# taconite/arah-release

Measured on AMD Instinct MI355X. Metric: rendered rays/sec, higher is better.
Workload: dtype f32 (operands as hi+lo f16 pairs on the f16 MFMA pipe, fp32 accumulate)

## Files before the change

arah_release_amd/csrc/arah_hip.hip:

```cpp
#include <hip/hip_runtime.h>
#include <stdint.h>
#include <stdlib.h>
#include <string.h>

#include <atomic>
#include <mutex>

#include "../../include/arah_hip.h"
#include "pointwise.hpp"
#include "mlp.hpp"

using namespace arah;

namespace {

constexpr float kRootThresh = 1e-5f;
constexpr int kSphereIters = 50;
constexpr float kSurfaceRange = 0.05f;
constexpr float kClampDist = 0.1f;
constexpr int kBroydenSteps = 50;
constexpr float kDvg = 1.0f;
constexpr int kMaxVerts = 6912;
constexpr int kKnnThreads = 1024;
constexpr int kMaxGrid = 512;
// ... 1863 lines not shown
    }
    append_ids(keep, i, list, count);
}

__global__ void k_joint_seam_out(int n, const float* xbest, const float* zbest, const float* err_best, const uint8_t* valid,
                                 float* x, float* z, uint8_t* conv) {
    const int i = blockIdx.x * blockDim.x + threadIdx.x;
    if (i >= n) return;
    x[(size_t)i * 3] = xbest[(size_t)i * 3];
    x[(size_t)i * 3 + 1] = xbest[(size_t)i * 3 + 1];
    x[(size_t)i * 3 + 2] = xbest[(size_t)i * 3 + 2];
    z[i] = zbest[i];
    conv[i] = (valid[i] != 0 && err_best[i] < kRootThresh) ? 1 : 0;
}

__global__ void k_trace_finalize(FrameDev fr, int n, const float* near_far, const float* xbest, const float* zbest,
                                 const float* err_best, float* points_hat_norm, uint8_t* conv, float* start,
                                 float* end) {
    const BodyConst bc = load_bc(fr);
    const int i = blockIdx.x * blockDim.x + threadIdx.x;
    if (i >= n) return;
    const float nr = near_far[i * 2], fa = near_far[i * 2 + 1];
    const float z = zbest[i];
    const bool c = (err_best[i] < kRootThresh) && (z >= nr) && (z <= fa);
    const V3 xn = normalize_pt(bc, V3{xbest[(size_t)i * 3], xbest[(size_t)i * 3 + 1], xbest[(size_t)i * 3 + 2]});
    points_hat_norm[(size_t)i * 3] = xn.x;
    points_hat_norm[(size_t)i * 3 + 1] = xn.y;
    points_hat_norm[(size_t)i * 3 + 2] = xn.z;
    conv[i] = c ? 1 : 0;
    start[i] = c ? z : nr;
    end[i] = fa;
}

#include "finish.hpp"

template <typename F>
__device__ __forceinline__ float jittered(F val, int i, int m, float t) {
    const float v = val(i);
    const float lower = i == 0 ? v : 0.5f * (v + val(i - 1));
    const float upper = i == m - 1 ? v : 0.5f * (val(i + 1) + v);
    return lower + (upper - lower) * t;
}

__global__ void k_sample_depths(int n, int S, int n_near, int n_far, const float* near_far, const uint8_t* conv,
                                const float* start, const float* end, const float* lin_s, const float* lin_near,
                                const float* lin_far, const float* rand_s, const float* rand_near,
                                const float* rand_far, float* z, uint8_t* mask) {
    const int i = blockIdx.x * blockDim.x + threadIdx.x;
    if (i >= n) return;
    const float st = start[i], en = end[i];
    float* zr = z + (size_t)i * S;
    uint8_t* mr = mask + (size_t)i * S;
    auto uni = [&](int s) { return st + (en - st) * lin_s[s]; };
    auto uni_j = [&](int s) { return rand_s ? jittered(uni, s, S, rand_s[(size_t)i * S + s]) : uni(s); };
    if (!conv[i] || (n_near <= 0 && n_far <= 0)) {
        for (int s = 0; s < S; ++s) {
            zr[s] = uni_j(s);
            mr[s] = 1;
        }
        return;
    }
    const int nc = n_near + 1 + n_far;
    const float base = st - kSurfaceRange;
    const float nb = near_far[i * 2];
    const float span = fmaxf(st - kSurfaceRange - nb, 1e-5f);
    auto surf = [&](int a) { return base + (kSurfaceRange * 2.0f) * lin_near[a]; };
    auto farv = [&](int b) { return nb + span * lin_far[b]; };
// ... 594 lines not shown
    w.u_Jinv = c.take<float>(N * 16);
    w.err_best_ray = c.take<float>(N);
    w.xbest_ray = c.take<float>(N * 3);
    w.zbest_ray = c.take<float>(N);
    w.o_xnorm = c.take<float>(N * 3);
    w.o_Tray = c.take<float>(N * 16);
    w.o_start = c.take<float>(N);
    w.o_end = c.take<float>(N);
    w.o_acc = c.take<float>(N);
    w.o_conv = c.take<uint8_t>(N);
    w.listA = c.take<int>(Q);
    w.listB = c.take<int>(Q);
    w.q_err = c.take<float>(Q);
    w.o_z = c.take<float>(Q);
    w.o_pts = c.take<float>(Q * 3);
    w.o_T = c.take<float>(Q * 16);
    w.o_mask = c.take<uint8_t>(Q);
    w.q_smask = c.take<uint8_t>(Q);
    w.shaded = c.take<f32x4>(Q);
    w.listC = c.take<int>(Q);
    w.listD = c.take<int>(Q);
    w.tcounts = c.take<int>(TC_COUNT);
    w.ray_tier = c.take<uint8_t>(N);
    w.bytes = align_up(c.off, 256);
    return w;
}

struct Knobs {
    int max_grid;
    int knn_group;
    int knn_below[3];
    int joint_bulk;
    int trace_bulk;
    int trace_small;
    bool train_b3;
    int canon_tier_wgs;
    int posed_canon;
};
inline const Knobs& knobs() {
    static const Knobs k = [] {
        auto env_int = [](const char* name, int dflt) {
            const char* e = getenv(name);
            return e ? atoi(e) : dflt;
        };
        Knobs v;
        const int g = env_int("ARAH_MAX_GRID", kMaxGrid);
        v.max_grid = g >= 1 && g <= kMaxGrid ? g : kMaxGrid;
        v.knn_group = env_int("ARAH_KNN_GROUP", 1);
        v.knn_below[0] = env_int("ARAH_KNN_WAVE_POINTS", 4096);
        v.knn_below[1] = env_int("ARAH_KNN_WAVE_RAYS", v.knn_group ? (1 << 30) : 32768);
        v.knn_below[2] = env_int("ARAH_KNN_WAVE_SAMPLES", 32768);
        v.joint_bulk = max(1, min(kBroydenSteps + 1, env_int("ARAH_JOINT_BULK_ITERS", 3)));
        v.trace_bulk = max(0, min(kSphereIters, env_int("ARAH_TRACE_BULK_STEPS", 24)));
        v.trace_small = env_int("ARAH_TRACE_SMALL", 4096);
        v.canon_tier_wgs = max(0, env_int("ARAH_CANON_TIER_WGS", 0));
        const char* ck = getenv("ARAH_CANON_KERNEL");
        v.posed_canon = !ck ? ARAH_CANON_KERNEL_WAVE : strcmp(ck, "tile") == 0 ? ARAH_CANON_KERNEL_TILE
                        : strcmp(ck, "wave_l2") == 0 ? ARAH_CANON_KERNEL_WAVE_L2 : ARAH_CANON_KERNEL_WAVE;
        const char* e = getenv("ARAH_TRAIN_ENGINE");
        v.train_b3 = !(e && strcmp(e, "fp32") == 0);
        return v;
    }();
    return k;
}

inline int grid_for(long long n_items, int per_block) {
    long long g = (n_items + per_block - 1) / per_block;
    if (g < 1) g = 1;
    const int cap = knobs().max_grid;
    if (g > cap) g = cap;
    return (int)g;
}

inline int check_launch() { return hipGetLastError() == hipSuccess ? ARAH_OK : ARAH_E_LAUNCH; }

inline int num_cus() {
    constexpr int kMaxDevices = 64;
    static std::atomic<int> cus[kMaxDevices];
    int dev = 0;
    if (hipGetDevice(&dev) != hipSuccess || dev < 0 || dev >= kMaxDevices) return 256;
    int v = cus[dev].load(std::memory_order_relaxed);
    if (v == 0) {
        if (hipDeviceGetAttribute(&v, hipDeviceAttributeMultiprocessorCount, dev) != hipSuccess || v <= 0) v = 256;
        cus[dev].store(v, std::memory_order_relaxed);
    }
    return v;
}
// ... 42 lines not shown
    if (done[dev].load(std::memory_order_relaxed)) return ARAH_OK;
    const int rc = setup_attributes_once();
    if (rc == ARAH_OK) done[dev].store(true, std::memory_order_release);
    return rc;
}

int setup_attributes_once() {
    bool failed = false;
    allow_lds(k_nearest_invlbs<SRC_POINTS>, kLdsKnn, failed);
    allow_lds(k_nearest_invlbs<SRC_RAYS>, kLdsKnn, failed);
    allow_lds(k_nearest_invlbs<SRC_SAMPLES>, kLdsKnn, failed);
    allow_lds(k_sdf_eval<false, false>, kLdsSdfFwd, failed);
    allow_lds(k_sdf_eval<false, true>, kLdsSdfFwd, failed);
    allow_lds(k_sdf_eval<true, false>, kLdsSdfGrad, failed);
    allow_lds(k_sdf_eval<true, true>, kLdsSdfGrad, failed);
    allow_lds(k_sdf_march<false>, kLdsSdfFwd, failed);
    allow_lds(k_sdf_march<true>, kLdsSdfFwd, failed);
    allow_lds(k_density<false>, kLdsSdfFwd, failed);
    allow_lds(k_density<true>, kLdsSdfFwd, failed);
    allow_lds(k_density<true, 8>, kLdsDensityWide, failed);
    allow_lds(k_sdf_lattice, kLdsDensityWide, failed);
    allow_lds(k_skin_eval, kLdsSkin, failed);
    allow_lds(k_skin_jac, kLdsSkin, failed);
    allow_lds(k_canon_solve<false>, kLdsCanonSolve, failed);
    allow_lds(k_canon_solve<true>, kLdsCanonSolve, failed);
    allow_lds((k_canon_wave<true, false>), kLdsCanonWave, failed);
    allow_lds((k_canon_wave<true, true>), kLdsCanonWave, failed);
    allow_lds((k_canon_wave<false, false>), kLdsCanonWave, failed);
    allow_lds((k_canon_wave<false, true>), kLdsCanonWave, failed);
    allow_lds(k_joint_iter<true, false>, kLdsJoint, failed);
    allow_lds(k_joint_iter<true, true>, kLdsJoint, failed);
    allow_lds(k_joint_iter<false, false>, kLdsJoint, failed);
    allow_lds(k_joint_iter<false, true>, kLdsJoint, failed);
    allow_lds(k_trace_finish<true>, kLdsTraceFinish, failed);
    allow_lds(k_trace_finish<false>, kLdsTraceFinish, failed);
    allow_lds(k_joint_finish<true>, kLdsJointFinish, failed);
    allow_lds(k_joint_finish<false>, kLdsJointFinish, failed);
    allow_lds(k_shade<false, false>, lds_shade<false>(), failed);
    allow_lds(k_shade<false, true>, lds_shade<false>(), failed);
    allow_lds(k_shade<true, false>, lds_shade<true>(), failed);
    allow_lds(k_shade<true, true>, lds_shade<true>(), failed);
    allow_lds((k_shade<false, true, true>), lds_shade_b3<false>(), failed);
    allow_lds((k_shade<true, true, true>), lds_shade_b3<true>(), failed);
    allow_lds((k_shade<false, false, false, true>), lds_shade<false>(), failed);
    allow_lds((k_shade<false, true, false, true>), lds_shade<false>(), failed);
    allow_lds((k_shade<true, false, false, true>), lds_shade<true>(), failed);
    allow_lds((k_shade<true, true, false, true>), lds_shade<true>(), failed);
    allow_lds((k_shade<false, true, true, true>), lds_shade_b3<false>(), failed);
    allow_lds((k_shade<true, true, true, true>), lds_shade_b3<true>(), failed);
    allow_lds(k_color_eval<false>, lds_color<false>(), failed);
    allow_lds(k_color_eval<true>, lds_color<true>(), failed);
    allow_lds(k_shade_train<false, false, false>, lds_shade_train<false>(), failed);
    allow_lds(k_shade_train<false, true, false>, lds_shade_train<false>(), failed);
    allow_lds(k_shade_train<true, false, false>, lds_shade_train<true>(), failed);
    allow_lds(k_shade_train<true, true, false>, lds_shade_train<true>(), failed);
    allow_lds(k_shade_train<false, false, true>, lds_shade_train<false>(), failed);
    allow_lds(k_shade_train<false, true, true>, lds_shade_train<false>(), failed);
    allow_lds(k_shade_train<true, false, true>, lds_shade_train<true>(), failed);
    allow_lds(k_shade_train<true, true, true>, lds_shade_train<true>(), failed);
    return failed ? ARAH_E_LAUNCH : ARAH_OK;
}


KnnData knn_of(const FrameDev& fd) {
    return KnnData{fd.knn.sorted4, fd.knn.spheres, reinterpret_cast<const GridInfo*>(fd.knn.grid), fd.knn.cells};
}

template <int SRC>
void launch_nearest(hipStream_t s, const FrameDev& fd, long long n_max, const float* pts, const RaySet& rs,
                    const float* depth, int n_steps, const int* list, const int* count, int n_direct, int* idx_out,
// ... 883 lines not shown
    int rc = run_broyden3(fd, w, tgt, CanonOut{x, T, w.q_err}, n, s, canon_kernel);
    if (rc) return rc;
    hipLaunchKernelGGL(k_broyden3_finalize, dim3((n + 255) / 256), dim3(256), 0, s, n, (const float*)w.q_err, err, conv);
    return check_launch();
}

static void joint_impl(const FrameDev& fd, Workspace& w, const RaySet& rs, int n, float* T, hipStream_t s) {
    int* cntB = w.counts + kNumCounts;
    const int gm = grid_for(n, kTile);
    hipLaunchKernelGGL(k_skin_jac, dim3(grid_for(n, 16)), dim3(kThreads), kLdsSkin, s, fd, (const float*)w.x0raw,
                       (const int*)w.listA, (const int*)&cntB[0], 0, w.jac_lbs, &w.ctr->n_skin_jac);
    LAUNCH_ENGINE(fd.split, (k_sdf_eval<true, true>), (k_sdf_eval<true, false>), dim3(gm), dim3(kThreads), kLdsSdfGrad, s,
                  fd, (const float*)w.xcur, (const int*)w.listA, (const int*)&cntB[0], 0, w.u_gx ,
                  (float*)nullptr, w.grad_sdf, w.spill, &w.ctr->n_sdf_fwd, &w.ctr->n_sdf_grad, 0);
    Broyden4State st{w.u_eval, w.u_step, w.u_gx, w.u_Jinv, w.err_best_ray, w.xbest_ray, w.zbest_ray, T};
    hipLaunchKernelGGL(k_joint_init, dim3(grid_for(n, 256)), dim3(256), 0, s, fd, st, rs, (const int*)w.listA,
                       (const int*)&cntB[0], (const float*)w.grad_sdf, (const float*)w.jac_lbs, (const float*)w.xcur,
                       (const float*)w.t, w.x0raw);
    const int bulk = knobs().joint_bulk;
    for (int it = 0; it < bulk; ++it) {
        int* lin = (it & 1) ? w.listB : w.listA;
        int* lout = (it & 1) ? w.listA : w.listB;
        if (it == 0)
            LAUNCH_ENGINE(fd.split, (k_joint_iter<true, true>), (k_joint_iter<true, false>), dim3(gm), dim3(kThreads),
                          kLdsJoint, s, fd, st, rs, (const int*)lin, (const int*)&cntB[it], lout, &cntB[it + 1],
                          &w.ctr->n_skin_fwd, &w.ctr->n_sdf_fwd);
        else
            LAUNCH_ENGINE(fd.split, (k_joint_iter<false, true>), (k_joint_iter<false, false>), dim3(gm), dim3(kThreads),
                          kLdsJoint, s, fd, st, rs, (const int*)lin, (const int*)&cntB[it], lout, &cntB[it + 1],
                          &w.ctr->n_skin_fwd, &w.ctr->n_sdf_fwd);
    }
    if (bulk <= kBroydenSteps) {
        const int* lin = (bulk & 1) ? w.listB : w.listA;
        const int gf = min(4 * num_cus(), max(1, (n + kFinTile - 1) / kFinTile));
        LAUNCH_ENGINE(fd.split, k_joint_finish<true>, k_joint_finish<false>, dim3(gf), dim3(kThreads), kLdsJointFinish, s, fd,
                      st, rs, lin, (const int*)&cntB[bulk], kBroydenSteps + 1 - bulk, &w.ctr->n_skin_fwd, &w.ctr->n_sdf_fwd);
    }
}

static int trace_impl(const ArahFrame* f, Workspace& w, const float* cam_loc, int32_t rays_per_cam,
                      const float* dirs, const float* near_far, int32_t n, int root_find_all, float* points_hat_norm,
                      float* T, uint8_t* conv, float* start, float* end, hipStream_t s, const uint8_t* skip = nullptr) {
    const FrameDev fd = to_dev(*f);
    const RaySet rs = make_rays(cam_loc, dirs, rays_per_cam);
    const int gb = (n + 255) / 256;
    int* cntA = w.counts;
    int* cntB = w.counts + kNumCounts;
    hipMemsetAsync(w.counts, 0, sizeof(int) * 3 * kNumCounts, s);
    hipMemsetAsync(w.nn_idx, 0xff, sizeof(int) * (size_t)n, s);
    hipLaunchKernelGGL(k_trace_begin, dim3(gb), dim3(256), 0, s, near_far, n, w.t, w.far, w.diverged, w.xcur, w.Tcur,
                       w.listA, &cntA[0], skip);
    TraceState ts{w.t, w.far, w.xcur, w.diverged};
    const int gm = grid_for(n, kTile);
    const int bulk = n <= knobs().trace_small ? 0 : knobs().trace_bulk;
    for (int it = 0; it < bulk; ++it) {
        int* lin = (it & 1) ? w.listB : w.listA;
        int* lout = (it & 1) ? w.listA : w.listB;
        launch_nearest<SRC_RAYS>(s, fd, n, (const float*)nullptr, rs, (const float*)w.t, 1, (const int*)lin,
                                 (const int*)&cntA[it], 0, w.nn_idx, w.xcur, w.Tcur, 0, &w.ctr->n_knn);
        LAUNCH_ENGINE(fd.split, k_sdf_march<true>, k_sdf_march<false>, dim3(gm), dim3(kThreads), kLdsSdfFwd, s, fd, ts,
                      (const int*)lin, (const int*)&cntA[it], lout, &cntA[it + 1], &w.ctr->n_sdf_fwd);
    }
    if (bulk < kSphereIters) {
        const int* lin = (bulk & 1) ? w.listB : w.listA;
        const int gf = min(4 * num_cus(), max(1, (n + kFinTile - 1) / kFinTile));
        LAUNCH_ENGINE(fd.split, k_trace_finish<true>, k_trace_finish<false>, dim3(gf), dim3(kThreads), kLdsTraceFinish, s, fd,
                      knn_of(fd), rs, ts, w.Tcur, w.nn_idx, lin, (const int*)&cntA[bulk], kSphereIters - bulk, &w.ctr->n_knn,
                      &w.ctr->n_sdf_fwd);
    }
    hipLaunchKernelGGL(k_joint_select, dim3(gb), dim3(256), 0, s, fd, n, (const float*)w.xcur, (const float*)w.Tcur,
                       (const float*)w.t, (const uint8_t*)w.diverged, root_find_all, w.x0raw, w.xbest_ray, w.zbest_ray, T,
                       w.err_best_ray, w.listA, &cntB[0]);
    joint_impl(fd, w, rs, n, T, s);
    hipLaunchKernelGGL(k_trace_finalize, dim3(gb), dim3(256), 0, s, fd, n, near_far, (const float*)w.xbest_ray,
                       (const float*)w.zbest_ray, (const float*)w.err_best_ray, points_hat_norm, conv, start, end);
    return check_launch();
}

int arah_trace(const ArahFrame* f, const float* cam_loc, int32_t rays_per_cam, const float* dirs,
               const float* near_far, int32_t n, int32_t root_find_all, float* points_hat_norm, float* T,
               uint8_t* conv, float* start, float* end, void* workspace, size_t wbytes, void* stream) {
    if (!f || n < 0 || !workspace) return ARAH_E_BADARG;
    if (n == 0) return ARAH_OK;
    if (!cam_loc || !dirs || !near_far || !points_hat_norm || !T || !conv || !start || !end) return ARAH_E_BADARG;
    Workspace w = carve(workspace, n, 1);
    if (wbytes < w.bytes) return ARAH_E_WORKSPACE;
    if (int arc = setup_attributes()) return arc;
    return trace_impl(f, w, cam_loc, rays_per_cam, dirs, near_far, n, root_find_all, points_hat_norm, T, conv, start,
                      end, reinterpret_cast<hipStream_t>(stream));
}

int arah_joint_root_find(const ArahFrame* f, const float* cam_loc, int32_t rays_per_cam, const float* dirs,
                         const uint8_t* valid, const float* x0, const float* z0, const float* T0, int32_t n, float* x,
                         float* z, float* T, uint8_t* conv, void* workspace, size_t wbytes, void* stream) {
    if (!f || n < 0 || !workspace) return ARAH_E_BADARG;
    if (n == 0) return ARAH_OK;
    if (!cam_loc || !dirs || !valid || !x0 || !z0 || !T0 || !x || !z || !T || !conv) return ARAH_E_BADARG;
    Workspace w = carve(workspace, n, 1);
    if (wbytes < w.bytes) return ARAH_E_WORKSPACE;
    if (int arc = setup_attributes()) return arc;
    hipStream_t s = reinterpret_cast<hipStream_t>(stream);
// ... 1334 lines not shown
```

arah_release_amd/csrc/finish.hpp:

```cpp
#pragma once

constexpr int kFinTile = 16;
constexpr size_t kLdsTraceFinish = (kFinTile * 4 * 2 + kFinTile * 16 + kFinTile * 8) * 4 + (size_t)kFinTile * kSdfLd * 4;
constexpr size_t kLdsJointFinish = (kFinTile * 4 * 3 + 24 * 16 + kFinTile * 2 + kFinTile * kLogitLd + 32) * 4 + (size_t)kFinTile * kSdfLd * 4;

template <bool SPLIT>
__global__ __launch_bounds__(kThreads, 4) void k_trace_finish(FrameDev fr, KnnData kd, RaySet rs, TraceState st, float* Tcur,
                                                            int* nn_idx, const int* list, const int* count, int steps_left,
                                                            unsigned long long* ctr_knn, unsigned long long* ctr_fwd) {
    const BodyConst bc = load_bc(fr);
    extern __shared__ __attribute__((aligned(16))) float smem[];
    float* xin = smem;
    float* outv = xin + kFinTile * 4;
    float* Tl = outv + kFinTile * 4;
    int* ids = reinterpret_cast<int*>(Tl + kFinTile * 16);
    float* tl = reinterpret_cast<float*>(ids + kFinTile);
    float* farl = tl + kFinTile;
    int* nnl = reinterpret_cast<int*>(farl + kFinTile);
    int* divl = nnl + kFinTile;
    int* s_live = divl + kFinTile;
    float* actA = reinterpret_cast<float*>(s_live + 3 * kFinTile);
    const int tid = threadIdx.x, wave = __builtin_amdgcn_readfirstlane(tid >> 6), lane = tid & 63;
    const int n = *count;
    const GridInfo g = *kd.grid;
    const float scale = sdf_scale(bc);
    int n_done = 0;
    for (int tile = blockIdx.x; tile * kFinTile < n; tile += gridDim.x) {
        __syncthreads();
        if (tid < kFinTile) {
            const int i = tile * kFinTile + tid;
            const int id = i < n ? list[i] : -1;
            ids[tid] = id;
            tl[tid] = id >= 0 ? st.t[id] : 0.f;
            farl[tid] = id >= 0 ? st.far[id] : 0.f;
            nnl[tid] = id >= 0 ? nn_idx[id] : -1;
            divl[tid] = 0;
        }
        for (int step = 0; step < steps_left; ++step) {
            __syncthreads();
            if (wave == 0) {
                const unsigned long long live = __ballot(lane < kFinTile && ids[lane] >= 0);
                n_done += __popcll(live);
                if (lane == 0) *s_live = live != 0ull;
            }
            __syncthreads();
            if (!*s_live) break;
            if (wave < 4) {
                const int s = wave * 4 + (lane >> 4);
                const int id = ids[s];
                if (id >= 0) {
                    const V3 p = ray_point(rs, id, tl[s]);
                    float best = 3.4e38f;
                    int bi = 0x7fffffff;
                    const int seed = nnl[s];
                    if (seed >= 0) {
                        const float dx = fr.verts_raw[seed * 3] - p.x, dy = fr.verts_raw[seed * 3 + 1] - p.y,
                                    dz = fr.verts_raw[seed * 3 + 2] - p.z;
                        best = dx * dx + dy * dy + dz * dz;
                        bi = seed;
                    }
                    bi = nearest_vertex_group16<kClusterSize>(kd, kd.sorted4, kd.spheres, g, p, best, bi, lane);
                    if ((lane & 15) == 0) {
                        float T[16];
                        vertex_transform(fr, bi, T);
                        const V3 y = V3{p.x - bc.trans[0], p.y - bc.trans[1], p.z - bc.trans[2]};
                        const V3 xh = normalize_pt(bc, inverse_affine_apply(T, y));
                        store_T(Tl + s * 16, T);
                        nnl[s] = bi;
                        reinterpret_cast<f32x4*>(xin)[s] = f32x4{xh.x, xh.y, xh.z, 0.f};
                    }
                } else if ((lane & 15) == 0) {
                    reinterpret_cast<f32x4*>(xin)[s] = f32x4{0.f, 0.f, 0.f, 0.f};
                }
            }
            __syncthreads();
            f32x4 dlast[kSdfMT][1];
            sdf_trunk<false, 1, SPLIT>(fr.sdf, xin, actA, kSdfLd, nullptr, dlast, wave, lane);
            sdf_head<SPLIT>(fr.sdf, actA, kSdfLd, outv, 4, tid, kFinTile);
            __syncthreads();
            if (tid < kFinTile) {
                const int id = ids[tid];
                if (id >= 0) {
                    const float sdf = outv[tid * 4] * scale;
                    const float march = fminf(fmaxf(sdf, -kClampDist), kClampDist);
                    bool div = false;
                    if (fabsf(march) > kRootThresh) {
                        const float t = tl[tid] + march;
                        tl[tid] = t;
                        div = t >= farl[tid];
                        divl[tid] = div ? 1 : 0;
                    }
                    const bool keep = !((fabsf(sdf) <= kRootThresh) || div);
                    if (!keep || step + 1 == steps_left) {
                        st.t[id] = tl[tid];
                        st.diverged[id] = divl[tid] ? 1 : 0;
                        const f32x4 xn = reinterpret_cast<const f32x4*>(xin)[tid];
                        st.xcur[(size_t)id * 3] = xn[0];
                        st.xcur[(size_t)id * 3 + 1] = xn[1];
                        st.xcur[(size_t)id * 3 + 2] = xn[2];
#pragma unroll
                        for (int c = 0; c < 4; ++c)
                            reinterpret_cast<f32x4*>(Tcur + (size_t)id * 16)[c] = reinterpret_cast<const f32x4*>(Tl + tid * 16)[c];
                        nn_idx[id] = nnl[tid];
                        ids[tid] = -1;
                    }
                }
            }
        }
    }
    if (tid == 0) {
        count_add(ctr_knn, n_done);
        count_add(ctr_fwd, n_done);
    }
}

template <bool SPLIT>
__global__ __launch_bounds__(kThreads, 4) void k_joint_finish(FrameDev fr, Broyden4State st, RaySet rs, const int* list,
                                                            const int* count, int iters_left, unsigned long long* ctr_skin,
                                                            unsigned long long* ctr_sdf) {
    const BodyConst bc = load_bc(fr);
    extern __shared__ __attribute__((aligned(16))) float smem[];
    constexpr int TW = kFinTile;
    float* xin = smem;
    float* xraw = xin + TW * 4;
    float* outv = xraw + TW * 4;
    float* sbones = outv + TW * 4;
    int* ids = reinterpret_cast<int*>(sbones + 24 * 16);
    int* s_live = ids + TW;
    float* logits = reinterpret_cast<float*>(s_live + TW);
    float* act = logits + TW * kLogitLd;
    const int tid = threadIdx.x, wave = __builtin_amdgcn_readfirstlane(tid >> 6), lane = tid & 63;
    const int n = *count;
    const float scale = sdf_scale(bc);
    int n_done = 0;
    for (int i = tid; i < 24 * 16; i += kThreads) sbones[i] = fr.bones[i];
    for (int tile = blockIdx.x; tile * TW < n; tile += gridDim.x) {
        __syncthreads();
        if (tid < TW) {
            const int i = tile * TW + tid;
            ids[tid] = i < n ? list[i] : -1;
        }
        for (int it = 0; it < iters_left; ++it) {
            __syncthreads();
            if (wave == 0) {
                const unsigned long long live = __ballot(lane < TW && ids[lane] >= 0);
                n_done += __popcll(live);
                if (lane == 0) *s_live = live != 0ull;
            }
            if (tid < TW) {
                const int id = ids[tid];
                f32x4 u = {0.f, 0.f, 0.f, 0.f};
                if (id >= 0) u = reinterpret_cast<const f32x4*>(st.ueval)[id];
                const V3 q = normalize_pt(bc, V3{u[0], u[1], u[2]});
                reinterpret_cast<f32x4*>(xin)[tid] = f32x4{q.x, q.y, q.z, 0.f};
                reinterpret_cast<f32x4*>(xraw)[tid] = u;
            }
            __syncthreads();
            if (!*s_live) break;
            skin_mlp<1>(fr.skin, xin, act, logits, wave, lane);
            f32x4 dlast[kSdfMT][1];
            sdf_trunk<false, 1, SPLIT>(fr.sdf, xin, act, kSdfLd, nullptr, dlast, wave, lane);
            sdf_head<SPLIT>(fr.sdf, act, kSdfLd, outv, 4, tid, TW);
            __syncthreads();
            if (tid < TW) {
                const int id = ids[tid];
                if (id >= 0) {
                    float T[16];
                    V3 xb;
                    const f32x4 u = reinterpret_cast<const f32x4*>(xraw)[tid];
                    skin_tail(logits + tid * kLogitLd, sbones, V3{u[0], u[1], u[2]}, T, xb);
                    const V3 p = ray_point(rs, id, u[3]);
                    float gnew[4] = {outv[tid * 4] * scale, xb.x - (p.x - bc.trans[0]), xb.y - (p.y - bc.trans[1]),
                                     xb.z - (p.z - bc.trans[2])};
                    float J[16], stp[4], gx[4], dg[4], dx[4];
#pragma unroll
                    for (int e = 0; e < 16; ++e) J[e] = st.Jinv[(size_t)id * 16 + e];
#pragma unroll
                    for (int r = 0; r < 4; ++r) {
                        dx[r] = st.step[(size_t)id * 4 + r];
                        const float gold = st.gx[(size_t)id * 4 + r];
                        dg[r] = gnew[r] - gold;
                        gx[r] = gold + dg[r];
                    }
                    const float err = sqrtf(gx[0] * gx[0] + gx[1] * gx[1] + gx[2] * gx[2] + gx[3] * gx[3]);
                    float eb = st.err_best[id];
                    if (err < eb) {
                        eb = err;
                        st.err_best[id] = err;
                        st.xbest[(size_t)id * 3] = u[0];
                        st.xbest[(size_t)id * 3 + 1] = u[1];
                        st.xbest[(size_t)id * 3 + 2] = u[2];
                        st.zbest[id] = u[3];
                        store_T(st.Tbest + (size_t)id * 16, T);
                    }
                    const bool keep = (eb > kRootThresh) && (err < kDvg);
                    if (keep) {
                        broyden_update<4>(J, dx, dg, gx, stp);
#pragma unroll
                        for (int r = 0; r < 4; ++r) st.gx[(size_t)id * 4 + r] = gx[r];
#pragma unroll
                        for (int e = 0; e < 16; ++e) st.Jinv[(size_t)id * 16 + e] = J[e];
                        reinterpret_cast<f32x4*>(st.step)[id] = f32x4{stp[0], stp[1], stp[2], stp[3]};
                        reinterpret_cast<f32x4*>(st.ueval)[id] = f32x4{u[0] + stp[0], u[1] + stp[1], u[2] + stp[2], u[3] + stp[3]};
                    } else {
                        ids[tid] = -1;
                    }
                }
            }
        }
    }
    if (tid == 0) {
        count_add(ctr_skin, n_done);
        count_add(ctr_sdf, n_done);
    }
}
```

Measured before the change: 11.43 million.

## Replace fixed-tile finish kernels with persistent resident-tile kernels that refill from a global queue

```diff
diff --git a/arah_release_amd/csrc/arah_hip.hip b/arah_release_amd/csrc/arah_hip.hip
--- a/arah_release_amd/csrc/arah_hip.hip
+++ b/arah_release_amd/csrc/arah_hip.hip
@@ -1919,7 +1919,7 @@
     end[i] = fa;
 }
 
-#include "finish.hpp"
+#include "resident.hpp"
 
 template <typename F>
 __device__ __forceinline__ float jittered(F val, int i, int m, float t) {
@@ -2580,7 +2580,6 @@
     int knn_below[3];
     int joint_bulk;
     int trace_bulk;
-    int trace_small;
     bool train_b3;
     int canon_tier_wgs;
     int posed_canon;
@@ -2598,9 +2597,8 @@
         v.knn_below[0] = env_int("ARAH_KNN_WAVE_POINTS", 4096);
         v.knn_below[1] = env_int("ARAH_KNN_WAVE_RAYS", v.knn_group ? (1 << 30) : 32768);
         v.knn_below[2] = env_int("ARAH_KNN_WAVE_SAMPLES", 32768);
-        v.joint_bulk = max(1, min(kBroydenSteps + 1, env_int("ARAH_JOINT_BULK_ITERS", 3)));
-        v.trace_bulk = max(0, min(kSphereIters, env_int("ARAH_TRACE_BULK_STEPS", 24)));
-        v.trace_small = env_int("ARAH_TRACE_SMALL", 4096);
+        v.joint_bulk = max(1, min(kBroydenSteps + 1, env_int("ARAH_JOINT_BULK_ITERS", 1)));
+        v.trace_bulk = max(0, min(kSphereIters, env_int("ARAH_TRACE_BULK_STEPS", 0)));
         v.canon_tier_wgs = max(0, env_int("ARAH_CANON_TIER_WGS", 0));
         const char* ck = getenv("ARAH_CANON_KERNEL");
         v.posed_canon = !ck ? ARAH_CANON_KERNEL_WAVE : strcmp(ck, "tile") == 0 ? ARAH_CANON_KERNEL_TILE
@@ -2709,10 +2707,10 @@
     allow_lds(k_joint_iter<true, true>, kLdsJoint, failed);
     allow_lds(k_joint_iter<false, false>, kLdsJoint, failed);
     allow_lds(k_joint_iter<false, true>, kLdsJoint, failed);
-    allow_lds(k_trace_finish<true>, kLdsTraceFinish, failed);
-    allow_lds(k_trace_finish<false>, kLdsTraceFinish, failed);
-    allow_lds(k_joint_finish<true>, kLdsJointFinish, failed);
-    allow_lds(k_joint_finish<false>, kLdsJointFinish, failed);
+    allow_lds(k_trace_resident<true>, kLdsTraceResident, failed);
+    allow_lds(k_trace_resident<false>, kLdsTraceResident, failed);
+    allow_lds(k_joint_resident<true>, kLdsJointResident, failed);
+    allow_lds(k_joint_resident<false>, kLdsJointResident, failed);
     allow_lds(k_shade<false, false>, lds_shade<false>(), failed);
     allow_lds(k_shade<false, true>, lds_shade<false>(), failed);
     allow_lds(k_shade<true, false>, lds_shade<true>(), failed);
@@ -3662,9 +3660,10 @@
     }
     if (bulk <= kBroydenSteps) {
         const int* lin = (bulk & 1) ? w.listB : w.listA;
-        const int gf = min(4 * num_cus(), max(1, (n + kFinTile - 1) / kFinTile));
-        LAUNCH_ENGINE(fd.split, k_joint_finish<true>, k_joint_finish<false>, dim3(gf), dim3(kThreads), kLdsJointFinish, s, fd,
-                      st, rs, lin, (const int*)&cntB[bulk], kBroydenSteps + 1 - bulk, &w.ctr->n_skin_fwd, &w.ctr->n_sdf_fwd);
+        const int gf = min((kJointResNT == 4 ? 1 : 2) * num_cus(), max(1, (n + kJointResTile - 1) / kJointResTile));
+        LAUNCH_ENGINE(fd.split, k_joint_resident<true>, k_joint_resident<false>, dim3(gf), dim3(kThreads), kLdsJointResident, s,
+                      fd, st, rs, lin, (const int*)&cntB[bulk], &w.counts[2 * kNumCounts + 1], bulk, &w.ctr->n_skin_fwd,
+                      &w.ctr->n_sdf_fwd);
     }
 }
 
@@ -3682,7 +3681,7 @@
                        w.listA, &cntA[0], skip);
     TraceState ts{w.t, w.far, w.xcur, w.diverged};
     const int gm = grid_for(n, kTile);
-    const int bulk = n <= knobs().trace_small ? 0 : knobs().trace_bulk;
+    const int bulk = knobs().trace_bulk;
     for (int it = 0; it < bulk; ++it) {
         int* lin = (it & 1) ? w.listB : w.listA;
         int* lout = (it & 1) ? w.listA : w.listB;
@@ -3693,10 +3692,10 @@
     }
     if (bulk < kSphereIters) {
         const int* lin = (bulk & 1) ? w.listB : w.listA;
-        const int gf = min(4 * num_cus(), max(1, (n + kFinTile - 1) / kFinTile));
-        LAUNCH_ENGINE(fd.split, k_trace_finish<true>, k_trace_finish<false>, dim3(gf), dim3(kThreads), kLdsTraceFinish, s, fd,
-                      knn_of(fd), rs, ts, w.Tcur, w.nn_idx, lin, (const int*)&cntA[bulk], kSphereIters - bulk, &w.ctr->n_knn,
-                      &w.ctr->n_sdf_fwd);
+        const int gf = min(2 * num_cus(), max(1, (n + kResTile - 1) / kResTile));
+        LAUNCH_ENGINE(fd.split, k_trace_resident<true>, k_trace_resident<false>, dim3(gf), dim3(kThreads), kLdsTraceResident, s,
+                      fd, knn_of(fd), rs, ts, w.Tcur, w.nn_idx, lin, (const int*)&cntA[bulk], &w.counts[2 * kNumCounts], bulk,
+                      &w.ctr->n_knn, &w.ctr->n_sdf_fwd);
     }
     hipLaunchKernelGGL(k_joint_select, dim3(gb), dim3(256), 0, s, fd, n, (const float*)w.xcur, (const float*)w.Tcur,
                        (const float*)w.t, (const uint8_t*)w.diverged, root_find_all, w.x0raw, w.xbest_ray, w.zbest_ray, T,
diff --git a/arah_release_amd/csrc/finish.hpp b/arah_release_amd/csrc/finish.hpp
--- a/arah_release_amd/csrc/finish.hpp
+++ /dev/null
@@ -1,216 +0,0 @@
-#pragma once
-
-constexpr int kFinTile = 16;
-constexpr size_t kLdsTraceFinish = (kFinTile * 4 * 2 + kFinTile * 16 + kFinTile * 8) * 4 + (size_t)kFinTile * kSdfLd * 4;
-constexpr size_t kLdsJointFinish = (kFinTile * 4 * 3 + 24 * 16 + kFinTile * 2 + kFinTile * kLogitLd + 32) * 4 + (size_t)kFinTile * kSdfLd * 4;
-
-template <bool SPLIT>
-__global__ __launch_bounds__(kThreads, 4) void k_trace_finish(FrameDev fr, KnnData kd, RaySet rs, TraceState st, float* Tcur,
-                                                            int* nn_idx, const int* list, const int* count, int steps_left,
-                                                            unsigned long long* ctr_knn, unsigned long long* ctr_fwd) {
-    const BodyConst bc = load_bc(fr);
-    extern __shared__ __attribute__((aligned(16))) float smem[];
-    float* xin = smem;
-    float* outv = xin + kFinTile * 4;
-    float* Tl = outv + kFinTile * 4;
-    int* ids = reinterpret_cast<int*>(Tl + kFinTile * 16);
-    float* tl = reinterpret_cast<float*>(ids + kFinTile);
-    float* farl = tl + kFinTile;
-    int* nnl = reinterpret_cast<int*>(farl + kFinTile);
-    int* divl = nnl + kFinTile;
-    int* s_live = divl + kFinTile;
-    float* actA = reinterpret_cast<float*>(s_live + 3 * kFinTile);
-    const int tid = threadIdx.x, wave = __builtin_amdgcn_readfirstlane(tid >> 6), lane = tid & 63;
-    const int n = *count;
-    const GridInfo g = *kd.grid;
-    const float scale = sdf_scale(bc);
-    int n_done = 0;
-    for (int tile = blockIdx.x; tile * kFinTile < n; tile += gridDim.x) {
-        __syncthreads();
-        if (tid < kFinTile) {
-            const int i = tile * kFinTile + tid;
-            const int id = i < n ? list[i] : -1;
-            ids[tid] = id;
-            tl[tid] = id >= 0 ? st.t[id] : 0.f;
-            farl[tid] = id >= 0 ? st.far[id] : 0.f;
-            nnl[tid] = id >= 0 ? nn_idx[id] : -1;
-            divl[tid] = 0;
-        }
-        for (int step = 0; step < steps_left; ++step) {
-            __syncthreads();
-            if (wave == 0) {
-                const unsigned long long live = __ballot(lane < kFinTile && ids[lane] >= 0);
-                n_done += __popcll(live);
-                if (lane == 0) *s_live = live != 0ull;
-            }
-            __syncthreads();
-            if (!*s_live) break;
-            if (wave < 4) {
-                const int s = wave * 4 + (lane >> 4);
-                const int id = ids[s];
-                if (id >= 0) {
-                    const V3 p = ray_point(rs, id, tl[s]);
-                    float best = 3.4e38f;
-                    int bi = 0x7fffffff;
-                    const int seed = nnl[s];
-                    if (seed >= 0) {
-                        const float dx = fr.verts_raw[seed * 3] - p.x, dy = fr.verts_raw[seed * 3 + 1] - p.y,
-                                    dz = fr.verts_raw[seed * 3 + 2] - p.z;
-                        best = dx * dx + dy * dy + dz * dz;
-                        bi = seed;
-                    }
-                    bi = nearest_vertex_group16<kClusterSize>(kd, kd.sorted4, kd.spheres, g, p, best, bi, lane);
-                    if ((lane & 15) == 0) {
-                        float T[16];
-                        vertex_transform(fr, bi, T);
-                        const V3 y = V3{p.x - bc.trans[0], p.y - bc.trans[1], p.z - bc.trans[2]};
-                        const V3 xh = normalize_pt(bc, inverse_affine_apply(T, y));
-                        store_T(Tl + s * 16, T);
-                        nnl[s] = bi;
-                        reinterpret_cast<f32x4*>(xin)[s] = f32x4{xh.x, xh.y, xh.z, 0.f};
-                    }
-                } else if ((lane & 15) == 0) {
-                    reinterpret_cast<f32x4*>(xin)[s] = f32x4{0.f, 0.f, 0.f, 0.f};
-                }
-            }
-            __syncthreads();
-            f32x4 dlast[kSdfMT][1];
-            sdf_trunk<false, 1, SPLIT>(fr.sdf, xin, actA, kSdfLd, nullptr, dlast, wave, lane);
-            sdf_head<SPLIT>(fr.sdf, actA, kSdfLd, outv, 4, tid, kFinTile);
-            __syncthreads();
-            if (tid < kFinTile) {
-                const int id = ids[tid];
-                if (id >= 0) {
-                    const float sdf = outv[tid * 4] * scale;
-                    const float march = fminf(fmaxf(sdf, -kClampDist), kClampDist);
-                    bool div = false;
-                    if (fabsf(march) > kRootThresh) {
-                        const float t = tl[tid] + march;
-                        tl[tid] = t;
-                        div = t >= farl[tid];
-                        divl[tid] = div ? 1 : 0;
-                    }
-                    const bool keep = !((fabsf(sdf) <= kRootThresh) || div);
-                    if (!keep || step + 1 == steps_left) {
-                        st.t[id] = tl[tid];
-                        st.diverged[id] = divl[tid] ? 1 : 0;
-                        const f32x4 xn = reinterpret_cast<const f32x4*>(xin)[tid];
-                        st.xcur[(size_t)id * 3] = xn[0];
-                        st.xcur[(size_t)id * 3 + 1] = xn[1];
-                        st.xcur[(size_t)id * 3 + 2] = xn[2];
-#pragma unroll
-                        for (int c = 0; c < 4; ++c)
-                            reinterpret_cast<f32x4*>(Tcur + (size_t)id * 16)[c] = reinterpret_cast<const f32x4*>(Tl + tid * 16)[c];
-                        nn_idx[id] = nnl[tid];
-                        ids[tid] = -1;
-                    }
-                }
-            }
-        }
-    }
-    if (tid == 0) {
-        count_add(ctr_knn, n_done);
-        count_add(ctr_fwd, n_done);
-    }
-}
-
-template <bool SPLIT>
-__global__ __launch_bounds__(kThreads, 4) void k_joint_finish(FrameDev fr, Broyden4State st, RaySet rs, const int* list,
-                                                            const int* count, int iters_left, unsigned long long* ctr_skin,
-                                                            unsigned long long* ctr_sdf) {
-    const BodyConst bc = load_bc(fr);
-    extern __shared__ __attribute__((aligned(16))) float smem[];
-    constexpr int TW = kFinTile;
-    float* xin = smem;
-    float* xraw = xin + TW * 4;
-    float* outv = xraw + TW * 4;
-    float* sbones = outv + TW * 4;
-    int* ids = reinterpret_cast<int*>(sbones + 24 * 16);
-    int* s_live = ids + TW;
-    float* logits = reinterpret_cast<float*>(s_live + TW);
-    float* act = logits + TW * kLogitLd;
-    const int tid = threadIdx.x, wave = __builtin_amdgcn_readfirstlane(tid >> 6), lane = tid & 63;
-    const int n = *count;
-    const float scale = sdf_scale(bc);
-    int n_done = 0;
-    for (int i = tid; i < 24 * 16; i += kThreads) sbones[i] = fr.bones[i];
-    for (int tile = blockIdx.x; tile * TW < n; tile += gridDim.x) {
-        __syncthreads();
-        if (tid < TW) {
-            const int i = tile * TW + tid;
-            ids[tid] = i < n ? list[i] : -1;
-        }
-        for (int it = 0; it < iters_left; ++it) {
-            __syncthreads();
-            if (wave == 0) {
-                const unsigned long long live = __ballot(lane < TW && ids[lane] >= 0);
-                n_done += __popcll(live);
-                if (lane == 0) *s_live = live != 0ull;
-            }
-            if (tid < TW) {
-                const int id = ids[tid];
-                f32x4 u = {0.f, 0.f, 0.f, 0.f};
-                if (id >= 0) u = reinterpret_cast<const f32x4*>(st.ueval)[id];
-                const V3 q = normalize_pt(bc, V3{u[0], u[1], u[2]});
-                reinterpret_cast<f32x4*>(xin)[tid] = f32x4{q.x, q.y, q.z, 0.f};
-                reinterpret_cast<f32x4*>(xraw)[tid] = u;
-            }
-            __syncthreads();
-            if (!*s_live) break;
-            skin_mlp<1>(fr.skin, xin, act, logits, wave, lane);
-            f32x4 dlast[kSdfMT][1];
-            sdf_trunk<false, 1, SPLIT>(fr.sdf, xin, act, kSdfLd, nullptr, dlast, wave, lane);
-            sdf_head<SPLIT>(fr.sdf, act, kSdfLd, outv, 4, tid, TW);
-            __syncthreads();
-            if (tid < TW) {
-                const int id = ids[tid];
-                if (id >= 0) {
-                    float T[16];
-                    V3 xb;
-                    const f32x4 u = reinterpret_cast<const f32x4*>(xraw)[tid];
-                    skin_tail(logits + tid * kLogitLd, sbones, V3{u[0], u[1], u[2]}, T, xb);
-                    const V3 p = ray_point(rs, id, u[3]);
-                    float gnew[4] = {outv[tid * 4] * scale, xb.x - (p.x - bc.trans[0]), xb.y - (p.y - bc.trans[1]),
-                                     xb.z - (p.z - bc.trans[2])};
-                    float J[16], stp[4], gx[4], dg[4], dx[4];
-#pragma unroll
-                    for (int e = 0; e < 16; ++e) J[e] = st.Jinv[(size_t)id * 16 + e];
-#pragma unroll
-                    for (int r = 0; r < 4; ++r) {
-                        dx[r] = st.step[(size_t)id * 4 + r];
-                        const float gold = st.gx[(size_t)id * 4 + r];
-                        dg[r] = gnew[r] - gold;
-                        gx[r] = gold + dg[r];
-                    }
-                    const float err = sqrtf(gx[0] * gx[0] + gx[1] * gx[1] + gx[2] * gx[2] + gx[3] * gx[3]);
-                    float eb = st.err_best[id];
-                    if (err < eb) {
-                        eb = err;
-                        st.err_best[id] = err;
-                        st.xbest[(size_t)id * 3] = u[0];
-                        st.xbest[(size_t)id * 3 + 1] = u[1];
-                        st.xbest[(size_t)id * 3 + 2] = u[2];
-                        st.zbest[id] = u[3];
-                        store_T(st.Tbest + (size_t)id * 16, T);
-                    }
-                    const bool keep = (eb > kRootThresh) && (err < kDvg);
-                    if (keep) {
-                        broyden_update<4>(J, dx, dg, gx, stp);
-#pragma unroll
-                        for (int r = 0; r < 4; ++r) st.gx[(size_t)id * 4 + r] = gx[r];
-#pragma unroll
-                        for (int e = 0; e < 16; ++e) st.Jinv[(size_t)id * 16 + e] = J[e];
-                        reinterpret_cast<f32x4*>(st.step)[id] = f32x4{stp[0], stp[1], stp[2], stp[3]};
-                        reinterpret_cast<f32x4*>(st.ueval)[id] = f32x4{u[0] + stp[0], u[1] + stp[1], u[2] + stp[2], u[3] + stp[3]};
-                    } else {
-                        ids[tid] = -1;
-                    }
-                }
-            }
-        }
-    }
-    if (tid == 0) {
-        count_add(ctr_skin, n_done);
-        count_add(ctr_sdf, n_done);
-    }
-}
diff --git a/arah_release_amd/csrc/resident.hpp b/arah_release_amd/csrc/resident.hpp
--- /dev/null
+++ b/arah_release_amd/csrc/resident.hpp
@@ -0,0 +1,324 @@
+#pragma once
+
+constexpr int kResTile = kTile;
+constexpr size_t kLdsTraceResident = (kResTile * 4 * 2 + kResTile * 16 + kResTile * 8) * 4 + (size_t)kResTile * kSdfLd * 4;
+
+#ifndef ARAH_JOINT_RES_NT
+#define ARAH_JOINT_RES_NT 2
+#endif
+constexpr int kJointResNT = ARAH_JOINT_RES_NT;
+constexpr int kJointResTile = 16 * kJointResNT;
+constexpr size_t kLdsJointResident =
+    (kJointResTile * (4 * 3 + 3 + 4 * 2 + 16) + 24 * 16 + 32 + kJointResTile * kLogitLd) * 4 + (size_t)kJointResTile * kSdfLd * 4;
+static_assert(kJointResNT == 2 || kJointResNT == 4, "loop B's resident tile is 32 or 64 rays");
+static_assert((kJointResTile * kLogitLd) % 4 == 0, "the activation tile stays 16-byte aligned");
+
+template <bool SPLIT>
+__global__ __launch_bounds__(kThreads, 4) void k_trace_resident(FrameDev fr, KnnData kd, RaySet rs, TraceState st, float* Tcur,
+                                                              int* nn_idx, const int* list, const int* count, int* head,
+                                                              int steps0, unsigned long long* ctr_knn,
+                                                              unsigned long long* ctr_fwd) {
+    constexpr int TW = kResTile;
+    extern __shared__ __attribute__((aligned(16))) float smem[];
+    float* xin = smem;
+    float* outv = xin + TW * 4;
+    float* Tl = outv + TW * 4;
+    int* ids = reinterpret_cast<int*>(Tl + TW * 16);
+    float* tl = reinterpret_cast<float*>(ids + TW);
+    float* farl = tl + TW;
+    int* nnl = reinterpret_cast<int*>(farl + TW);
+    int* divl = nnl + TW;
+    int* stl = divl + TW;
+    int* ctrl = stl + TW;
+    float* actA = reinterpret_cast<float*>(ctrl + 2 * TW);
+    const int tid = threadIdx.x, wave = __builtin_amdgcn_readfirstlane(tid >> 6), lane = tid & 63;
+    const int n = *count;
+    int nl = 0;
+    bool dry = false;
+    int n_done = 0;
+    for (;;) {
+        if (!dry && nl < TW) {
+            const int want = TW - nl;
+            if (tid == 0) ctrl[0] = atomicAdd(head, want);
+            __syncthreads();
+            const int base = ctrl[0];
+            const int take = max(0, min(want, n - base));
+            dry = base + want >= n;
+            int tr = tid;
+            asm volatile("" : "+v"(tr));
+            if (tr < take) {
+                const int id = list[base + tr], s = nl + tr;
+                ids[s] = id;
+                tl[s] = st.t[id];
+                farl[s] = st.far[id];
+                nnl[s] = nn_idx[id];
+                divl[s] = 0;
+                stl[s] = steps0;
+            }
+            nl += take;
+        }
+        if (nl == 0) break;
+        __syncthreads();
+        n_done += nl;
+        const bool narrow = nl <= 16;
+        const int cols = narrow ? 16 : TW;
+        for (int s = wave * 4 + (lane >> 4); s < cols; s += kWaves * 4) {
+            if (s < nl) {
+                const BodyConst bc = load_bc(fr);
+                const GridInfo g = *kd.grid;
+                const int id = ids[s];
+                const V3 p = ray_point(rs, id, tl[s]);
+                float best = 3.4e38f;
+                int bi = 0x7fffffff;
+                const int seed = nnl[s];
+                if (seed >= 0) {
+                    const float dx = fr.verts_raw[seed * 3] - p.x, dy = fr.verts_raw[seed * 3 + 1] - p.y,
+                                dz = fr.verts_raw[seed * 3 + 2] - p.z;
+                    best = dx * dx + dy * dy + dz * dz;
+                    bi = seed;
+                }
+                bi = nearest_vertex_group16<kClusterSize>(kd, kd.sorted4, kd.spheres, g, p, best, bi, lane);
+                if ((lane & 15) == 0) {
+                    float T[16];
+                    vertex_transform(fr, bi, T);
+                    const V3 y = V3{p.x - bc.trans[0], p.y - bc.trans[1], p.z - bc.trans[2]};
+                    const V3 xh = normalize_pt(bc, inverse_affine_apply(T, y));
+                    store_T(Tl + s * 16, T);
+                    nnl[s] = bi;
+                    reinterpret_cast<f32x4*>(xin)[s] = f32x4{xh.x, xh.y, xh.z, 0.f};
+                }
+            } else if ((lane & 15) == 0) {
+                reinterpret_cast<f32x4*>(xin)[s] = f32x4{0.f, 0.f, 0.f, 0.f};
+            }
+        }
+        __syncthreads();
+        int lm = lane;
+        asm volatile("" : "+v"(lm));
+        if (narrow) {
+            f32x4 dlast[kSdfMT][1];
+            sdf_trunk<false, 1, SPLIT>(fr.sdf, xin, actA, kSdfLd, nullptr, dlast, wave, lm);
+        } else {
+            f32x4 dlast[kSdfMT][kNT];
+            sdf_trunk<false, kNT, SPLIT>(fr.sdf, xin, actA, kSdfLd, nullptr, dlast, wave, lm);
+        }
+        sdf_head<SPLIT>(fr.sdf, actA, kSdfLd, outv, 4, tid, cols);
+        __syncthreads();
+        if (wave == 0) {
+            int ln = lane;
+            asm volatile("" : "+v"(ln));
+            const bool live = ln < nl;
+            bool keep = false;
+            int id = -1, nn = -1, dv = 0, sc = 0;
+            float t = 0.f, fa = 0.f;
+            if (live) {
+                id = ids[ln];
+                t = tl[ln];
+                fa = farl[ln];
+                nn = nnl[ln];
+                dv = divl[ln];
+                sc = stl[ln] + 1;
+                const float sdf = outv[ln * 4] * sdf_scale(load_bc(fr));
+                const float march = fminf(fmaxf(sdf, -kClampDist), kClampDist);
+                bool div = false;
+                if (fabsf(march) > kRootThresh) {
+                    t = t + march;
+                    div = t >= fa;
+                    dv = div ? 1 : 0;
+                }
+                keep = !((fabsf(sdf) <= kRootThresh) || div) && sc < kSphereIters;
+                if (!keep) {
+                    st.t[id] = t;
+                    st.diverged[id] = dv ? 1 : 0;
+                    const f32x4 xn = reinterpret_cast<const f32x4*>(xin)[ln];
+                    st.xcur[(size_t)id * 3] = xn[0];
+                    st.xcur[(size_t)id * 3 + 1] = xn[1];
+                    st.xcur[(size_t)id * 3 + 2] = xn[2];
+#pragma unroll
+                    for (int c = 0; c < 4; ++c)
+                        reinterpret_cast<f32x4*>(Tcur + (size_t)id * 16)[c] = reinterpret_cast<const f32x4*>(Tl + ln * 16)[c];
+                    nn_idx[id] = nn;
+                }
+            }
+            const unsigned long long m = __ballot(keep);
+            const int dst = __builtin_amdgcn_mbcnt_hi((unsigned)(m >> 32), __builtin_amdgcn_mbcnt_lo((unsigned)m, 0u));
+            __builtin_amdgcn_wave_barrier();
+            if (keep) {
+                ids[dst] = id;
+                tl[dst] = t;
+                farl[dst] = fa;
+                nnl[dst] = nn;
+                divl[dst] = dv;
+                stl[dst] = sc;
+            }
+            if (lane == 0) ctrl[1] = __popcll(m);
+        }
+        __syncthreads();
+        nl = ctrl[1];
+    }
+    if (tid == 0 && n_done) {
+        count_add(ctr_knn, n_done);
+        count_add(ctr_fwd, n_done);
+    }
+}
+
+template <bool SPLIT>
+__global__ __launch_bounds__(kThreads, kJointResNT == 4 ? 2 : 4) void k_joint_resident(FrameDev fr, Broyden4State st, RaySet rs,
+                                                                                     const int* list, const int* count, int* head,
+                                                                                     int iters0, unsigned long long* ctr_skin,
+                                                                                     unsigned long long* ctr_sdf) {
+    constexpr int TW = kJointResTile, NT = kJointResNT;
+    extern __shared__ __attribute__((aligned(16))) float smem[];
+    float* xin = smem;
+    float* xraw = xin + TW * 4;
+    float* outv = xraw + TW * 4;
+    float* stepl = outv + TW * 4;
+    float* gxl = stepl + TW * 4;
+    float* Jl = gxl + TW * 4;
+    float* ebl = Jl + TW * 16;
+    int* ids = reinterpret_cast<int*>(ebl + TW);
+    int* itl = ids + TW;
+    int* ctrl = itl + TW;
+    float* sbones = reinterpret_cast<float*>(ctrl + 32);
+    float* logits = sbones + 24 * 16;
+    float* act = logits + TW * kLogitLd;
+    const int tid = threadIdx.x, wave = __builtin_amdgcn_readfirstlane(tid >> 6), lane = tid & 63;
+    const int n = *count;
+    int nl = 0;
+    bool dry = false;
+    int n_done = 0;
+    for (int i = tid; i < 24 * 16; i += kThreads) sbones[i] = fr.bones[i];
+    for (;;) {
+        if (!dry && nl < TW) {
+            const int want = TW - nl;
+            if (tid == 0) ctrl[0] = atomicAdd(head, want);
+            __syncthreads();
+            const int base = ctrl[0];
+            const int take = max(0, min(want, n - base));
+            dry = base + want >= n;
+            int tr = tid;
+            asm volatile("" : "+v"(tr));
+            if (tr < take) {
+                const int id = list[base + tr], s = nl + tr;
+                ids[s] = id;
+                itl[s] = iters0;
+                reinterpret_cast<f32x4*>(xraw)[s] = reinterpret_cast<const f32x4*>(st.ueval)[id];
+                const f32x4 sp = reinterpret_cast<const f32x4*>(st.step)[id];
+                const f32x4 gv = reinterpret_cast<const f32x4*>(st.gx)[id];
+#pragma unroll
+                for (int r = 0; r < 4; ++r) {
+                    stepl[r * TW + s] = sp[r];
+                    gxl[r * TW + s] = gv[r];
+                }
+#pragma unroll
+                for (int c = 0; c < 4; ++c) {
+                    const f32x4 jv = reinterpret_cast<const f32x4*>(st.Jinv + (size_t)id * 16)[c];
+#pragma unroll
+                    for (int r = 0; r < 4; ++r) Jl[(c * 4 + r) * TW + s] = jv[r];
+                }
+                ebl[s] = st.err_best[id];
+            }
+            nl += take;
+        }
+        if (nl == 0) break;
+        __syncthreads();
+        n_done += nl;
+        const bool narrow = nl <= 16;
+        const int cols = narrow ? 16 : TW;
+        if (tid < cols) {
+            f32x4 x = {0.f, 0.f, 0.f, 0.f};
+            if (tid < nl) {
+                const f32x4 u = reinterpret_cast<const f32x4*>(xraw)[tid];
+                const V3 q = normalize_pt(load_bc(fr), V3{u[0], u[1], u[2]});
+                x = f32x4{q.x, q.y, q.z, 0.f};
+            }
+            reinterpret_cast<f32x4*>(xin)[tid] = x;
+        }
+        __syncthreads();
+        int lm = lane;
+        asm volatile("" : "+v"(lm));
+        if (narrow) {
+            skin_mlp<1>(fr.skin, xin, act, logits, wave, lm);
+            f32x4 dlast[kSdfMT][1];
+            sdf_trunk<false, 1, SPLIT>(fr.sdf, xin, act, kSdfLd, nullptr, dlast, wave, lm);
+        } else {
+            skin_mlp<NT>(fr.skin, xin, act, logits, wave, lm);
+            f32x4 dlast[kSdfMT][NT];
+            sdf_trunk<false, NT, SPLIT>(fr.sdf, xin, act, kSdfLd, nullptr, dlast, wave, lm);
+        }
+        sdf_head<SPLIT>(fr.sdf, act, kSdfLd, outv, 4, tid, cols);
+        __syncthreads();
+        if (wave == 0) {
+            int ln = lane;
+            asm volatile("" : "+v"(ln));
+            const bool live = ln < nl;
+            bool keep = false;
+            int id = -1, ic = 0;
+            float J[16] = {}, stp[4] = {}, gx[4] = {}, eb = 0.f;
+            f32x4 u = {0.f, 0.f, 0.f, 0.f};
+            if (live) {
+                const BodyConst bc = load_bc(fr);
+                const float scale = sdf_scale(bc);
+                id = ids[ln];
+                ic = itl[ln] + 1;
+                float T[16];
+                V3 xb;
+                u = reinterpret_cast<const f32x4*>(xraw)[ln];
+                skin_tail(logits + ln * kLogitLd, sbones, V3{u[0], u[1], u[2]}, T, xb);
+                const V3 p = ray_point(rs, id, u[3]);
+                float gnew[4] = {outv[ln * 4] * scale, xb.x - (p.x - bc.trans[0]), xb.y - (p.y - bc.trans[1]),
+                                 xb.z - (p.z - bc.trans[2])};
+                float dg[4], dx[4];
+#pragma unroll
+                for (int r = 0; r < 4; ++r) {
+                    dx[r] = stepl[r * TW + ln];
+                    const float gold = gxl[r * TW + ln];
+                    dg[r] = gnew[r] - gold;
+                    gx[r] = gold + dg[r];
+                }
+                const float err = sqrtf(gx[0] * gx[0] + gx[1] * gx[1] + gx[2] * gx[2] + gx[3] * gx[3]);
+                eb = ebl[ln];
+                if (err < eb) {
+                    eb = err;
+                    st.err_best[id] = err;
+                    st.xbest[(size_t)id * 3] = u[0];
+                    st.xbest[(size_t)id * 3 + 1] = u[1];
+                    st.xbest[(size_t)id * 3 + 2] = u[2];
+                    st.zbest[id] = u[3];
+                    store_T(st.Tbest + (size_t)id * 16, T);
+                }
+                keep = (eb > kRootThresh) && (err < kDvg) && ic < kBroydenSteps + 1;
+                __builtin_amdgcn_sched_barrier(0);
+                if (keep) {
+#pragma unroll
+                    for (int e = 0; e < 16; ++e) J[e] = Jl[e * TW + ln];
+                    broyden_update<4>(J, dx, dg, gx, stp);
+#pragma unroll
+                    for (int r = 0; r < 4; ++r) u[r] += stp[r];
+                }
+            }
+            const unsigned long long m = __ballot(keep);
+            const int dst = __builtin_amdgcn_mbcnt_hi((unsigned)(m >> 32), __builtin_amdgcn_mbcnt_lo((unsigned)m, 0u));
+            __builtin_amdgcn_wave_barrier();
+            if (keep) {
+                ids[dst] = id;
+                itl[dst] = ic;
+                ebl[dst] = eb;
+                reinterpret_cast<f32x4*>(xraw)[dst] = u;
+#pragma unroll
+                for (int r = 0; r < 4; ++r) {
+                    stepl[r * TW + dst] = stp[r];
+                    gxl[r * TW + dst] = gx[r];
+                }
+#pragma unroll
+                for (int e = 0; e < 16; ++e) Jl[e * TW + dst] = J[e];
+            }
+            if (lane == 0) ctrl[1] = __popcll(m);
+        }
+        __syncthreads();
+        nl = ctrl[1];
+    }
+    if (tid == 0 && n_done) {
+        count_add(ctr_skin, n_done);
+        count_add(ctr_sdf, n_done);
+    }
+}
```

Result: slower. 10.94 million (-4.3%).
